# kskjs1203/SevenNet_finetuning

Hardware: AMD Instinct MI355X
Metric: atoms/sec energy+force, SevenNet-0 lmax=2, 97,336-atom box @1 GPU (higher is better)
Workload: dtype f32 (MLP / linear products on bf16 MFMA pieces: bf16x6 fwd, bf16x3 bwd); 1 GPU; SevenNet-0 energy+force+virial, 97,336-atom periodic Si box (23^3 cells), 1 GPU; total_atoms=97336, scaling=weak, atoms_per_rank=97336, edges_per_rank=2725408, parallelism=single

## Files before the change

sevennet_finetuning_amd/csrc/api.cpp:

```cpp
#include <hip/hip_runtime.h>

#include <algorithm>
#include <cmath>
#include <cstdio>
#include <cstdlib>
#include <cstring>
#include <fstream>
#include <map>
#include <memory>
#include <sstream>
#include <string>
#include <vector>

#include "../../include/e3gnn.h"
#include "bias_row.h"
#include "cg_tables.h"
#include "d3.h"
#include "dbuf.h"
#include "fcn_act.h"
#include "generic.h"
#include "train_ops.h"
#include "common.h"
#include "fused.h"
#include "gtp.h"
#include "minijson.h"
#include "node.h"
#include "neighbor.h"
#include "tgemm.h"
#include "tp.h"

using namespace e3gnn;

namespace {

thread_local std::string g_err;

int fail(int code, const std::string& msg) {
  g_err = msg;
  return code;
}

bool trace_errors() {
  static int on = [] {
    const char* v = std::getenv("E3GNN_TRACE_ERRORS");
    return v && v[0] == '1';
  }();
  return on;
}
void trace_point(const char* where) {
  if (!trace_errors()) return;
  hipError_t e = hipPeekAtLastError();
  if (e != hipSuccess) std::fprintf(stderr, "[e3gnn] sticky HIP error %d (%s) at %s\n", (int)e,
                                    hipGetErrorString(e), where);
}

#define HIPCHK(expr)                                                                          \
  do {                                                                                        \
    hipError_t _e = (expr);                                                                   \
    if (_e != hipSuccess)                                                                     \
      return fail(E3GNN_ERR_HIP, std::string(#expr) + ": " + hipGetErrorString(_e));         \
  } while (0)

struct Irr {
  int mul, l;
};
using Irreps = std::vector<Irr>;

Irreps parse_irreps(const std::string& s) {
  Irreps out;
  std::stringstream ss(s);
  std::string term;
  while (std::getline(ss, term, '+')) {
    const auto x = term.find('x');
    out.push_back({std::stoi(term.substr(0, x)), std::stoi(term.substr(x + 1))});
  }
  return out;
}
int irreps_dim(const Irreps& ir) {
  int d = 0;
  for (auto& i : ir) d += i.mul * (2 * i.l + 1);
  return d;
}
// ... 18 lines not shown
  std::memcpy(&x, &u, 4);
  return x;
}

struct LinBlock {
  int l, K, N, in_off, out_off, w_off, wt_off;
};
struct Linear {
  std::vector<LinBlock> blocks;
  DBuf W, WT;
  std::vector<float> W_h, WT_h;
  int din = 0, dout = 0;
};

struct PairBlock {
  int l, N, out_off, K1, off1, K2, off2, w_off;
  int64_t wb_off;
};
struct LinPair {
  std::vector<PairBlock> blocks;
  DBuf W;
  DBuf Wb;
  bool ok = false;
};

}

struct e3gnn_model {
  int device = 0;
  int nsp = 0, nlayer = 0;
  int family = 0;
  int kcode(int t) const { return 3 * family + (t == 0 ? 0 : (t == nlayer - 1 ? 2 : 1)); }
  std::vector<GateDims> gdims;
  int max_dx = 0, max_dg = 0;
  float cutoff = 5.f, r_on = 4.5f;
  int raw_sh = 0;
  std::vector<Irreps> irreps;
  std::vector<Irreps> gin, mid;
  std::vector<int> W;
  std::vector<float> denom;
  DBuf coeffs, embed, readout_v, scale, shift;
  std::vector<std::unique_ptr<Linear>> sc, si1, si2;
  std::vector<DBuf> b_si1, b_si2;
  bool fcn = false;
  FcnDims fcnd{};
  DBuf fcn_w;
  std::vector<std::unique_ptr<LinPair>> nl_si1, nl_si1t, nl_si2t, nl_fwd, nl_bwd;
  struct Mlp {
    DBuf w0, w1, w2, w0t, w1t, w2t;
    DBuf w1p, w2p, w2q, w2r;
    DBuf w2b;
    DBuf w2d;
    DBuf w2v;
    DBuf w1b, w1tb, w0tb;
  };
  std::vector<Mlp> mlp;
  GenModel* gen = nullptr;
  ~e3gnn_model() {
    if (gen) gen_free(gen);
  }
};

namespace {

struct Stat {
  double ms = 0, flops = 0, bytes = 0;
  int64_t launches = 0;
};
struct Pending {
  int cls;
  hipEvent_t a, b;
  double flops, bytes;
};
const char* kClassNames[] = {"graph_build", "edge_embed",  "node_linear", "radial_mlp_fwd",
                             "tp_fwd",      "gate_fwd",    "readout",     "gate_bwd",
                             "tp_bwd",      "radial_mlp_bwd", "gather_src", "edge_force",
                             "atom_force",  "embed",
                             "conv_fwd.first", "conv_fwd.mid", "conv_fwd.last",
                             "conv_bwd_x.first", "conv_bwd_x.mid", "conv_bwd_x.last"};
enum Cls {
  C_GRAPH,
  C_EMBED_EDGE,
  C_LINEAR,
  C_MLP_FWD,
  C_TP_FWD,
  C_GATE_FWD,
  C_READOUT,
  C_GATE_BWD,
  C_TP_BWD,
  C_MLP_BWD,
  C_GATHER,
  C_EDGE_FORCE,
  C_ATOM_FORCE,
  C_EMBED_NODE,
  C_CONV_FWD,
  C_CONV_BWD_X = C_CONV_FWD + 3,
  C_NCLS = C_CONV_BWD_X + 3
};
static_assert(sizeof(kClassNames) / sizeof(kClassNames[0]) == C_NCLS, "class names");

double tp_flops_per_edge(int code) { return fused_kind_tp_flops(code); }

}

struct e3gnn_ctx {
  e3gnn_model* m;
// ... 306 lines not shown
bool check_paths(int code, const Irreps& x, int lmax_out) {
  struct Ins {
    int l1, l2, l3, mul, xoff;
  };
  const auto P = kind_paths(code);
  int DX = 0, W = 0, DM = 0;
  if (P.empty() || !fused_kind_dims(code, &DX, &W, &DM)) return false;
  std::vector<Ins> ins;
  int xoff = 0;
  for (auto& i : x) {
    for (int l2 = 0; l2 <= 2; ++l2)
      for (int l3 = std::abs(i.l - l2); l3 <= i.l + l2; ++l3)
        if (l3 <= lmax_out) ins.push_back({i.l, l2, l3, i.mul, xoff});
    xoff += i.mul * (2 * i.l + 1);
  }
  if (ins.size() != P.size()) return false;
  std::vector<int> moff(ins.size());
  int off = 0;
  for (int l3 = 0; l3 <= 2; ++l3)
    for (size_t k = 0; k < ins.size(); ++k)
      if (ins[k].l3 == l3) {
        moff[k] = off;
        off += ins[k].mul * (2 * l3 + 1);
      }
  if (off != DM) return false;
  int woff = 0;
  for (size_t k = 0; k < ins.size(); ++k) {
    const PathDef& p = P[k];
    if (p.l1 != ins[k].l1 || p.l2 != ins[k].l2 || p.l3 != ins[k].l3 || p.mul != ins[k].mul ||
        p.xoff != ins[k].xoff || p.woff != woff || p.moff != moff[k])
      return false;
    woff += ins[k].mul;
  }
  return woff == W && xoff == DX;
}

}

namespace {
template <int A, int B, int C>
void dense_cg(float* out) {
  using T = CG<A, B, C>;
  std::memset(out, 0, sizeof(float) * (2 * A + 1) * (2 * B + 1) * (2 * C + 1));
  for (int q = 0; q < T::n; ++q)
    out[(T::e[q].i * (2 * B + 1) + T::e[q].j) * (2 * C + 1) + T::e[q].k] = T::e[q].c;
}
MlpW mlp_ptrs(const e3gnn_model* m, int t) {
  const auto& mm = m->mlp[t];
  return MlpW{mm.w0.f(),  mm.w1.f(),  mm.w2.f(),  mm.w2t.f(),
              mm.w1p.f(), mm.w2p.f(), mm.w2q.f(), mm.w2r.f(),
              static_cast<const uint16_t*>(mm.w2b.p),
              static_cast<const uint16_t*>(mm.w2d.p),
              static_cast<const uint16_t*>(mm.w2v.p),
              static_cast<const uint16_t*>(mm.w1b.p),
              static_cast<const uint16_t*>(mm.w1tb.p),
              static_cast<const uint16_t*>(mm.w0tb.p)};
}

}

namespace {
GenGraph gen_graph(e3gnn_ctx* c) {
  return GenGraph{c->n, c->nl, c->E, c->type.i(), c->nbr.i(), c->vec.f(), c->row_ptr.i(),
                  c->src_ptr.i(), c->src_perm.i(), c->err.i()};
}

int fused_family(const minijson::Value& man) {
  if (const char* g = std::getenv("E3GNN_GENERIC"); g && g[0] == '1') return -1;
  if (man.has("is_parity") && man["is_parity"].boolean()) return -1;
  const int lmax = man.has("lmax_edge") ? (int)man["lmax_edge"].num()
                                        : (man.has("lmax") ? (int)man["lmax"].num() : 2);
  if (lmax != 2) return -1;
  if (man.has("self_connection_type") && man["self_connection_type"].str() != "linear") return -1;
  if (!man.has("cutoff_function") || man["cutoff_function"]["name"].str() != "XPLOR") return -1;
  if (man.has("readout") && man["readout"].has("type") && man["readout"]["type"].str() != "linear") {
    const auto& ro = man["readout"];
    if (ro["type"].str() != "fcn" || !ro.has("hidden") || !ro.has("act") || !ro.has("act_norm")) return -1;
    const auto& h = ro["hidden"].arr();
    if (h.size() < 1 || h.size() > (size_t)FCN_MAX_HIDDEN) return -1;
    for (auto& w : h)
      if (w.num() < 1 || w.num() > FCN_MAX_WIDTH || w.num() != std::floor(w.num())) return -1;
    bool known = false;
    for (int k = 0; k < FCN_ACT_KINDS; ++k) known = known || ro["act"].str() == fcn_act_names()[k];
    if (!known) return -1;
  }
  const int L = (int)man["num_convolution_layer"].num();
  if (L < 2) return -1;
  if (man.has("weight_nn_hidden_neurons")) {
    const auto& h = man["weight_nn_hidden_neurons"].arr();
    if (h.size() != 2 || (int)h[0].num() != 64 || (int)h[1].num() != 64) return -1;
  }
  if (man.has("radial_basis") && man["radial_basis"].has("num") && (int)man["radial_basis"]["num"].num() != 8)
    return -1;
  const auto& ir = man["irreps_manual"].arr();
  if ((int)ir.size() != L + 1) return -1;
  Irreps first, mid, last;
  try {
    first = merged(parse_irreps(ir[0].str()));
    mid = merged(parse_irreps(ir[1].str()));
    last = merged(parse_irreps(ir[L].str()));
  } catch (...) {
    return -1;
  }
  if (first.size() != 1 || first[0].l != 0 || last.size() != 1 || last[0].l != 0) return -1;
  for (int t = 1; t < L; ++t)
    if (ir[t].str() != ir[1].str()) return -1;
// ... 267 lines not shown
              for (int q = 0; q < 4; ++q)
                for (int t = 0; t < 4; ++t)
                  o[(size_t)n * 64 + g * 16 + q * 4 + t] = a[(size_t)(16 * q + 4 * g + t) * N + n];
          return o;
        };
        std::vector<float> q2((size_t)W * 64);
        for (int cb = 0; cb < W / 16; ++cb)
          for (int bh = 0; bh < 4; ++bh)
            for (int g = 0; g < 4; ++g)
              for (int c = 0; c < 16; ++c)
                for (int sx = 0; sx < 4; ++sx)
                  q2[((size_t)(cb * 4 + bh) * 64 + g * 16 + c) * 4 + sx] =
                      a2[(size_t)(16 * bh + c) * W + 16 * cb + 4 * sx + g];
        std::vector<float> r2((size_t)W * 64);
        for (int cb = 0; cb < W / 16; ++cb)
          for (int bh = 0; bh < 4; ++bh)
            for (int g = 0; g < 4; ++g)
              for (int c = 0; c < 16; ++c)
                for (int r = 0; r < 4; ++r)
                  r2[((size_t)(cb * 4 + bh) * 64 + g * 16 + c) * 4 + r] =
                      a2[(size_t)(16 * bh + c) * W + 16 * cb + 4 * g + r];
        auto bsplit = [](const std::vector<float>& a, int N) {
          std::vector<float> o((size_t)N * 64 * 3 / 2);
          uint16_t* oh = reinterpret_cast<uint16_t*>(o.data());
          for (int cb = 0; cb < N / 16; ++cb)
            for (int m2 = 0; m2 < 2; ++m2)
              for (int g = 0; g < 4; ++g)
                for (int c = 0; c < 16; ++c)
                  for (int t = 0; t < 8; ++t) {
                    float v = a[(size_t)(16 * (2 * m2 + t / 4) + 4 * g + t % 4) * N + 16 * cb + c];
                    for (int pc = 0; pc < 3; ++pc) {
                      const uint16_t hb = bf16_rne(v);
                      oh[((((size_t)cb * 3 + pc) * 2 + m2) * 64 + g * 16 + c) * 8 + t] = hb;
                      v -= bf16_to_f32(hb);
                    }
                  }
          return o;
        };
        const std::vector<float> b2 = bsplit(a2, W);
        {
          const auto a0 = scaled(w0, 8, 64, s0, false);
          std::vector<float> a1t((size_t)64 * 64), a0t((size_t)64 * 16, 0.f);
          for (int i = 0; i < 64; ++i)
            for (int j = 0; j < 64; ++j) a1t[(size_t)j * 64 + i] = a1[(size_t)i * 64 + j];
          for (int n = 0; n < 8; ++n)
            for (int k = 0; k < 64; ++k) a0t[(size_t)k * 16 + n] = a0[(size_t)n * 64 + k];
          if (upload(mm.w1b, bsplit(a1, 64)) != hipSuccess || upload(mm.w1tb, bsplit(a1t, 64)) != hipSuccess ||
              upload(mm.w0tb, bsplit(a0t, 16)) != hipSuccess)
            throw std::runtime_error("upload mlp (w1b)");
        }
        const std::vector<int> cols = bwd_w_block_cols(m->kcode(t));
        if ((int)cols.size() * 16 != W || cols.size() % 2)
          throw std::runtime_error("dE/dw block order does not cover the weights");
        std::vector<float> d2((size_t)W * 64 * 3 / 2);
        uint16_t* d2h = reinterpret_cast<uint16_t*>(d2.data());
        for (size_t P = 0; P < cols.size() / 2; ++P)
          for (int bh = 0; bh < 4; ++bh)
            for (int g = 0; g < 4; ++g)
              for (int c = 0; c < 16; ++c)
                for (int t8 = 0; t8 < 8; ++t8) {
                  const int col = t8 < 4 ? cols[2 * P] + 4 * g + t8 : cols[2 * P + 1] + 4 * g + t8 - 4;
                  float v = a2[(size_t)(16 * bh + c) * W + col];
                  for (int pc = 0; pc < 3; ++pc) {
                    const uint16_t hb = bf16_rne(v);
                    d2h[(((P * 3 + pc) * 4 + bh) * 64 + g * 16 + c) * 8 + t8] = hb;
                    v -= bf16_to_f32(hb);
                  }
                }
        if (upload(mm.w2d, d2) != hipSuccess) throw std::runtime_error("upload mlp (w2d)");
        {
          std::vector<float> v2(b2.size());
          const size_t blk = (size_t)64 * 16 * 3 / 2;
          for (size_t k = 0; k < cols.size(); ++k)
            std::memcpy(v2.data() + k * blk, b2.data() + (size_t)(cols[k] / 16) * blk, blk * 4);
          if (upload(mm.w2v, v2) != hipSuccess) throw std::runtime_error("upload mlp (w2v)");
        }
        if (W % 16 || upload(mm.w1p, kperm(a1, 64)) != hipSuccess ||
            upload(mm.w2p, kperm(a2, W)) != hipSuccess || upload(mm.w2q, q2) != hipSuccess ||
            upload(mm.w2r, r2) != hipSuccess ||
            upload(mm.w2b, b2) != hipSuccess)
          throw std::runtime_error("upload mlp (packed)");
      }
      trace_point("load:mlp");
    }
  } catch (const std::exception& ex) {
    fail(E3GNN_ERR_IO, std::string("model load: ") + ex.what());
    return nullptr;
  }
  trace_point("load:exit");
  (void)hipGetLastError();
  return m.release();
}

void e3gnn_free(e3gnn_model* m) { delete m; }

int e3gnn_model_info(const e3gnn_model* m, int* num_species, float* cutoff, int* num_layers,
                     int* comm_size) {
  if (!m) return fail(E3GNN_ERR_ARG, "null model");
  if (num_species) *num_species = m->nsp;
  if (cutoff) *cutoff = m->cutoff;
  if (num_layers) *num_layers = m->nlayer;
  if (comm_size) {
    if (m->gen) {
      int d = 0;
      for (int t = 1; t <= m->nlayer; ++t) d = std::max(d, gen_feature_dim(m->gen, t));
      *comm_size = d;
    } else {
      *comm_size = irreps_dim(m->irreps[1]);
    }
  }
  return E3GNN_OK;
}

int64_t e3gnn_gemm_workspace_floats(int n, const e3gnn_gemm_desc* d) {
  if (n < 0 || (n > 0 && !d)) return -1;
  int64_t w = 0;
  for (int i = 0; i < n; ++i) {
    const int sp = tg_splits(d[i].m, d[i].n, (int64_t)d[i].k + d[i].k2);
    if (sp > 1) w += (int64_t)sp * d[i].m * d[i].n;
  }
  return w;
}

static int gemm_prob(const e3gnn_gemm_desc& q, int i, TgProb& p) {
  if (q.m < 0 || q.n < 0 || q.k < 0 || q.k2 < 0 || (q.m > 0 && q.n > 0 && (!q.c || (q.k > 0 && (!q.a || !q.b)) ||
                                                                      (q.k2 > 0 && (!q.a2 || !q.b2)))))
    return fail(E3GNN_ERR_ARG, "e3gnn_gemm_grouped: bad problem " + std::to_string(i));
  if (q.beta != 0 && q.beta != 1) return fail(E3GNN_ERR_ARG, "e3gnn_gemm_grouped: beta must be 0 or 1");
// ... 1877 lines not shown
```

sevennet_finetuning_amd/csrc/fused.h:

```cpp
#pragma once
#include <hip/hip_runtime.h>
#include <cstdint>

namespace e3gnn {

struct MlpW {
  const float* w0;
  const float* w1;
  const float* w2;
  const float* w2t;
  const float* w1p;
  const float* w2p;
  const float* w2q;
  const float* w2r;
  const uint16_t* w2b;
  const uint16_t* w2d;
  const uint16_t* w2v;
  const uint16_t* w1b;
  const uint16_t* w1tb;
  const uint16_t* w0tb;
};

struct FusedArgs {
  const int* row_ptr;
  const int* center;
  const int* nbr;
  const float* emb;
  const float* Y;
  const float* h;
  float* agg;
  const float* gagg;
  const int* src_ptr;
  const int* src_perm;
  float* dh;
  float* dxc;
  float* dgu;
  float* demb;
  MlpW W;
  int n_centers;
  int n_edges;
  int n_nodes;
  float denom;
  int c_begin, c_end, node_begin, node_end;
};

hipError_t launch_conv_fwd(int kind, const FusedArgs& a, hipStream_t s);
hipError_t launch_conv_bwd_ls(int kind, const FusedArgs& a, hipStream_t s);
hipError_t launch_conv_bwd_nbr_last(int kind, const FusedArgs& a, hipStream_t s);

}
```

sevennet_finetuning_amd/csrc/fused.hip:

```cpp
#include "cg_tables.h"
#include "common.h"
#include "fused.h"
#include "tp.h"

#include <type_traits>


namespace e3gnn {
namespace {

typedef float f32x4 __attribute__((ext_vector_type(4)));

template <int N, int I = 0, class F>
constexpr void sfor_host(F&& f) {
  if constexpr (I < N) {
    f(std::integral_constant<int, I>{});
    sfor_host<N, I + 1>(f);
  }
}
template <int N, int I = 0, class F>
__device__ __forceinline__ void sfor(F&& f) {
  if constexpr (I < N) {
    f(std::integral_constant<int, I>{});
    sfor<N, I + 1>(f);
  }
}

__device__ __forceinline__ constexpr int yoff(int l) { return l == 0 ? 0 : (l == 1 ? 1 : 4); }
__device__ __forceinline__ constexpr int KH(int s) { return 16 * (s >> 2) + (s & 3); }

__device__ __forceinline__ void phase() { __builtin_amdgcn_sched_barrier(0); }

#ifndef E3GNN_STAMPS_FWD
#define E3GNN_STAMPS_FWD 0
#endif
#ifdef E3GNN_STAMPS
__device__ unsigned long long* g_stamp_buf = nullptr;
#define STAMP_N 8
#define STAMP_DECL                               \
  unsigned long long st_acc[STAMP_N] = {0, 0, 0, 0, 0, 0, 0, 0}; \
  unsigned long long st_t = __builtin_amdgcn_s_memtime(), st_t0 = st_t;
#define STAMP(k)                                          \
  do {                                                    \
    const unsigned long long st_now = __builtin_amdgcn_s_memtime(); \
    st_acc[k] += st_now - st_t;                           \
    st_t = st_now;                                        \
  } while (0)
#define STAMP_FLUSH(wave)                                                   \
  do {                                                                      \
    if (g_stamp_buf && lane == 0) {                                         \
      st_acc[7] = __builtin_amdgcn_s_memtime() - st_t0;                     \
      for (int k_ = 0; k_ < STAMP_N; ++k_) g_stamp_buf[(int64_t)(wave) * STAMP_N + k_] = st_acc[k_]; \
    }                                                                       \
  } while (0)
#else
#define STAMP_DECL
// ... 676 lines not shown
    mlp_chain<CX3>(R, b, lane, m);
  }

  f32x4 dh1[4];
  {
    f32x4 da2[4];
#pragma unroll
    for (int bb = 0; bb < 4; ++bb)
#pragma unroll
      for (int r = 0; r < 4; ++r) da2[bb][r] = dh2[bb][r] * act_grad(m.a2[bb][r]);
    Op3 dq;
    split_h2(da2, dq);
#pragma unroll
    for (int bi = 0; bi < 4; ++bi) {
      phase();
      Op3 wq;
      load_w2b(wq, R.w1tb, lane, 16 * bi);
      dh1[bi] = CX3 ? w2_block3<false>(dq, wq) : w2_block<false>(dq, wq);
    }
  }
  f32x4 de;
  {
    f32x4 da1[4];
#pragma unroll
    for (int q = 0; q < 4; ++q)
#pragma unroll
      for (int t = 0; t < 4; ++t) da1[q][t] = dh1[q][t] * act_grad(m.a1[q][t]);
    Op3 dq, wq;
    split_h2(da1, dq);
    load_w2b(wq, R.w0tb, lane, 0);
    de = CX3 ? w2_block3<false>(dq, wq) : w2_block<false>(dq, wq);
  }
  if (g < 2 && er >= 0) {
    if (dold) {
#pragma unroll
      for (int r = 0; r < 4; ++r) demb[(int64_t)er * 8 + 4 * g + r] = dold[r] + de[r];
    } else {
#pragma unroll
      for (int r = 0; r < 4; ++r) demb[(int64_t)er * 8 + 4 * g + r] += de[r];
    }
  }
}
__device__ __forceinline__ void mlp_bwd_chain(const WRes& R, const float* __restrict__ emb, int e0,
                                              int end, int lane, const f32x4 (&dh2)[4],
                                              float* __restrict__ demb, const float* dold = nullptr,
                                              const float* bk = nullptr, const f32x4* a2k = nullptr) {
  const int e = e0 + (lane & 15);
  mlp_bwd_chain_ids(R, emb, e < end ? e : -1, lane, dh2, demb, dold, bk, a2k);
}

#ifndef E3GNN_DH2_X3
#define E3GNN_DH2_X3 1
#endif
constexpr int LS_BLK = 6144;
constexpr int LS_PAIR_W = 2 * LS_BLK;
constexpr int LS_PAIR_D = 12288;

__device__ __forceinline__ void dh2_pair_g2(f32x4 (&dh2)[2][4], const float (&dp)[2][4], const float (&dr)[2][4],
                                            bool two, __amdgpu_buffer_rsrc_t w2d, int pair, int lane) {
  bf16x8 d[2][2];
#pragma unroll
  for (int u = 0; u < 2; ++u) {
    float v[8];
#pragma unroll
    for (int t = 0; t < 8; ++t) v[t] = t < 4 ? dp[u][t] : dr[u][t - 4];
    split2x8(v, d[u]);
  }
  bf16x8 a[4][2];
#pragma unroll
  for (int bh = 0; bh < 4; ++bh)
#pragma unroll
    for (int pc = 0; pc < 2; ++pc)
      a[bh][pc] = __builtin_bit_cast(
          bf16x8, __builtin_amdgcn_raw_buffer_load_b128(w2d, lane * 16, pair * LS_PAIR_D + (pc * 4 + bh) * 1024, 0));
#pragma unroll
  for (int bh = 0; bh < 4; ++bh) {
#pragma unroll
    for (int u = 0; u < 2; ++u) {
      if (u == 1 && !two) break;
      dh2[u][bh] = mfma16(a[bh][1], d[u][0], dh2[u][bh]);
      dh2[u][bh] = mfma16(a[bh][0], d[u][1], dh2[u][bh]);
      dh2[u][bh] = mfma16(a[bh][0], d[u][0], dh2[u][bh]);
    }
  }
}

constexpr bool NBR_DH2_BF16 = E3GNN_DH2_X3 != 0;
template <class L>
__global__ __launch_bounds__(256) __attribute__((amdgpu_waves_per_eu(2, 2))) void k_conv_bwd_nbr(
    const int* __restrict__ src_ptr, const int* __restrict__ src_perm, const int* __restrict__ center,
    const float* __restrict__ emb, const float* __restrict__ Y, const float* __restrict__ h,
    const float* __restrict__ gagg, MlpW W, float* __restrict__ dh, float* __restrict__ dgu, int n_centers,
    int r_begin, int r_end, float* __restrict__ demb) {
  __shared__ __attribute__((aligned(16))) float lds[4][L::DX];
  const int wid = threadIdx.x >> 6;
  const int jn = __builtin_amdgcn_readfirstlane(r_begin + blockIdx.x * 4 + wid);
  if (jn >= r_end) return;
  float* dacc = lds[wid];
  const int lane = threadIdx.x & 63, g = lane >> 4, col = lane & 15;
  const int qb = src_ptr[jn], qe = src_ptr[jn + 1];
  const WRes R = make_wres(W, L::W);
  const __amdgpu_buffer_rsrc_t Rx = rsrc_bytes(h + (int64_t)jn * L::DX, L::DX * 4);
  const __amdgpu_buffer_rsrc_t Rg = rsrc_bytes(gagg, (int64_t)n_centers * L::DM * 4);
  for (int t = lane; t < L::DX; t += 64) dacc[t] = 0.f;
  const RowSel rsel = row_scatter_sel(col);
  const int own = row_scatter_own(col);

  for (int q0 = qb; q0 < qe; q0 += 32) {
// ... 119 lines not shown
                }
              }
              pin<4 * D1>(dx);
              wcur[0] = wnxt[0];
              wcur[1] = wnxt[1];
              ++nb;
            }
          });
          phase();
          {
            constexpr int NV = 4 * D1;
            static_assert(NV % 8 == 4, "batches of 16, 8, then 4");
            float* da = dacc + XOFF + (16 * jj + 4 * g) * D1;
            if constexpr (NV >= 16) da[own] += row_scatter16<16>(dx, rsel);
            if constexpr (NV % 16 >= 8) da[NV / 16 * 16 + (own & 7)] += row_scatter16<8>(dx + NV / 16 * 16, rsel);
            da[NV / 8 * 8 + (own & 3)] += row_scatter16<4>(dx + NV / 8 * 8, rsel);
          }
        }
      }
    });

#pragma unroll
    for (int u = 0; u < 2; ++u) {
      if (u == 1 && !two) break;
      phase();
      float d[8];
#pragma unroll
      for (int q = 0; q < 8; ++q) d[q] = sum_rows4(dYa[u][q + 1]);
      if (g == 0 && er[u] >= 0) {
        const float s3 = 1.7320508075688772f, s5 = 2.23606797749979f, c15 = s3 * s5;
        const float is3 = 0.57735026918962576f;
        const float ux = y[u][1] * is3, uy = y[u][2] * is3, uz = y[u][3] * is3;
        const float gx = s3 * d[0] + c15 * (uz * d[3] + uy * d[4]) - s5 * ux * d[5] - c15 * ux * d[7];
        const float gy = s3 * d[1] + c15 * (ux * d[4] + uz * d[6]) + 2.f * s5 * uy * d[5];
        const float gz = s3 * d[2] + c15 * (ux * d[3] + uy * d[6]) - s5 * uz * d[5] + c15 * uz * d[7];
        float* o = dgu + (int64_t)er[u] * 3;
        o[0] = gu_old[u][0] + gx;
        o[1] = gu_old[u][1] + gy;
        o[2] = gu_old[u][2] + gz;
      }
      phase();
      mlp_bwd_chain_ids(R, emb, er[u], lane, dh2[u], demb, de_old[u]);
    }
  }
  phase();
  __builtin_amdgcn_s_waitcnt(0);
  float* dhj = dh + (int64_t)jn * L::DX;
  for (int t = lane; t < L::DX; t += 64) dhj[t] = dacc[t];
}


constexpr int LS_WPC = E3GNN_BWD_W_X3 ? 2 : 3;
constexpr int LS_DPC = E3GNN_DH2_X3 ? 2 : 3;
constexpr int LS_IBLK = LS_WPC * 2048;
constexpr int LS_IW = 2 * LS_IBLK;
constexpr int LS_IMG = LS_IW + LS_DPC * 4096;

template <int NPC = 3>
__device__ __forceinline__ void lds_op3(Op3& o, const char* blk, int lane) {
#pragma unroll
  for (int pc = 0; pc < NPC; ++pc)
#pragma unroll
    for (int m = 0; m < 2; ++m)
      o.v[pc][m] = *reinterpret_cast<const bf16x8*>(blk + ((pc * 2 + m) * 64 + lane) * 16);
}

__device__ __forceinline__ void dh2_pair(f32x4 (&dh2)[4], const float (&da)[4], const float (&db)[4],
                                         const char* pimg, int lane) {
  if constexpr (E3GNN_DH2_X3) {
    bf16x8 d[2];
    {
      float v[8];
#pragma unroll
      for (int t = 0; t < 8; ++t) v[t] = t < 4 ? da[t] : db[t - 4];
      split2x8(v, d);
    }
    bf16x8 a[4][2];
#pragma unroll
    for (int bh = 0; bh < 4; ++bh)
#pragma unroll
      for (int pc = 0; pc < 2; ++pc)
        a[bh][pc] = *reinterpret_cast<const bf16x8*>(pimg + ((pc * 4 + bh) * 64 + lane) * 16);
    phase();
#pragma unroll
    for (int bh = 0; bh < 4; ++bh) {
      dh2[bh] = mfma16(a[bh][1], d[0], dh2[bh]);
      dh2[bh] = mfma16(a[bh][0], d[1], dh2[bh]);
      dh2[bh] = mfma16(a[bh][0], d[0], dh2[bh]);
    }
    return;
  }
  bf16x8 d[3];
  {
    float v[8];
#pragma unroll
    for (int t = 0; t < 8; ++t) v[t] = t < 4 ? da[t] : db[t - 4];
    split3x8(v, d);
  }
  constexpr int I[6] = {2, 1, 0, 1, 0, 0}, J[6] = {0, 1, 2, 0, 1, 0};
#pragma unroll
  for (int bh = 0; bh < 4; ++bh) {
    bf16x8 a[3];
#pragma unroll
    for (int pc = 0; pc < 3; ++pc)
      a[pc] = *reinterpret_cast<const bf16x8*>(pimg + ((pc * 4 + bh) * 64 + lane) * 16);
#pragma unroll
    for (int q = 0; q < 6; ++q) dh2[bh] = mfma16(a[I[q]], d[J[q]], dh2[bh]);
  }
}

__device__ __forceinline__ int ls_tiles(const int* __restrict__ row_ptr, int cb, int c_end) {
  int T = 0;
#pragma unroll
  for (int w = 0; w < 4; ++w) {
    const int cc = cb + w;
    if (cc < c_end) T = max(T, (row_ptr[cc + 1] - row_ptr[cc] + 15) >> 4);
  }
  return __builtin_amdgcn_readfirstlane(T);
}

template <class L>
struct BwdLsWaves {
  static constexpr int v = L::KIND == 0 ? 3 : 2;
};
constexpr int LS_WPG = 4;
template <class L>
struct LsTwoImages {
  static constexpr bool lean = LS_WPC == 2 && LS_DPC == 2;
  static constexpr int OFF0 = L::KIND == 1 ? L::P[0].mul : 0;
  static constexpr int DMS = L::DM - OFF0;
  static constexpr int bytes = LS_WPG * DMS * 4 + 2 * LS_IMG;
  static constexpr bool v = lean && BwdLsWaves<L>::v * bytes <= 163840;
};
template <int P>
__device__ __forceinline__ void ls_prio() { __builtin_amdgcn_s_setprio(P); }
template <class L>
__global__ __launch_bounds__(64 * LS_WPG) __attribute__((amdgpu_waves_per_eu(BwdLsWaves<L>::v, BwdLsWaves<L>::v))) void k_conv_bwd_ls(
    const int* __restrict__ row_ptr, const int* __restrict__ nbr, const float* __restrict__ emb,
    const float* __restrict__ Y, const float* __restrict__ h, const float* __restrict__ gagg, MlpW W,
    float* __restrict__ dxc, float* __restrict__ dgu, float* __restrict__ demb, int c_begin,
    int c_end, int n_nodes) {
  constexpr int NBLK = L::W / 16, NPAIR = NBLK / 2;
  static_assert(NBLK % 2 == 0, "weight blocks come in pairs");
  constexpr int WPG = LS_WPG, NT = 64 * WPG;
  constexpr int NWP = LS_IW / 16, NW = NWP / NT, NST = LS_IMG / 16 / NT, PB = LS_IBLK / 16;
  static_assert(LS_IMG / 16 % NT == 0 && NWP % NT == 0 && PB % 64 == 0, "staging pieces per thread");
  constexpr bool TWO = LsTwoImages<L>::v;
  constexpr bool KEEP = BwdLsWaves<L>::v == 2;
  constexpr int OFF0 = TWO ? LsTwoImages<L>::OFF0 : 0, DMS = L::DM - OFF0;
  static_assert(!TWO || (L::P[0].l1 == 0 && L::P[0].l2 == 0 && L::P[0].l3 == 0 && L::P[0].moff == 0 &&
                         OFF0 % 4 == 0), "path 0 is the 0e x 0e -> 0e slice at the row start");
  __shared__ __attribute__((aligned(16))) float smem[WPG * DMS + (TWO ? 2 : 1) * LS_IMG / 4];
  const int tid = threadIdx.x, wid = __builtin_amdgcn_readfirstlane(tid >> 6), lane = tid & 63, g = lane >> 4, col = lane & 15;
  const int cb = c_begin + blockIdx.x * WPG;
  const int c = cb + wid;
  const bool valid = c < c_end;
  const int beg = valid ? row_ptr[c] : 0, end = valid ? row_ptr[c + 1] : 0;
  const int T = ls_tiles(row_ptr, cb, c_end);
  float* dacc = smem + wid * DMS - OFF0;
  char* img = reinterpret_cast<char*>(smem + WPG * DMS);
  if (valid && end > beg) {
    const float4* s4 = reinterpret_cast<const float4*>(gagg + (int64_t)c * L::DM + OFF0);
    float4* d4 = reinterpret_cast<float4*>(dacc + OFF0);
    for (int k = lane; k < DMS / 4; k += 64) d4[k] = s4[k];
  }
  int rb = 0;
  const __amdgpu_buffer_rsrc_t Rg0 =
      rsrc_bytes(gagg + (valid ? (int64_t)c * L::DM : 0), valid ? (int64_t)OFF0 * 4 : 0);
  const WRes R = make_wres(W, L::W);
  const __amdgpu_buffer_rsrc_t Rx = rsrc_bytes(h, (int64_t)n_nodes * L::DX * 4);
  f32x4 st[NST];
  auto issue = [&](int P) {
    auto wsrc = [&](int idx) { return (idx / PB) * LS_BLK + (idx % PB) * 16; };
#pragma unroll
    for (int i = 0; i < NW; ++i) st[i] = ldw4(R.w2v, wsrc(tid + NT * i), P * LS_PAIR_W);
#pragma unroll
    for (int i = NW; i < NST; ++i) st[i] = ldw4(R.w2d, (tid + NT * i - NWP) * 16, P * LS_PAIR_D);
  };
  auto commit = [&]() {
    __syncthreads();
#pragma unroll
    for (int i = 0; i < NST; ++i) *reinterpret_cast<f32x4*>(img + (tid + NT * i) * 16) = st[i];
    __syncthreads();
  };
  constexpr bool STAMPED = std::is_same<L, LayerMid>::value && !E3GNN_STAMPS_FWD;
  STAMP_DECL
  issue(0);
  for (int t = 0; t < T; ++t) {
    if constexpr (STAMPED) STAMP(0);
    const int q0 = beg + 16 * t;
    const bool act = q0 < end;
    const int er = (act && q0 + col < end) ? q0 + col : -1;
    const int vx = (er >= 0 ? nbr[er] : 0) * L::DX * 4;
    float xpf[20];
    float g0pf[4];
    auto load_group = [&](auto Iq, int jq) {
      constexpr int D1q = 2 * Iq + 1;
      constexpr int XOq = iblock_xoff<L, Iq>();
      ldv<4 * D1q>(Rx, vx + 4 * g * D1q * 4, (XOq + 16 * jq * D1q) * 4, xpf);
      if constexpr (OFF0 > 0 && Iq == 0) ldv<4>(Rg0, 4 * g * 4, 16 * jq * 4, g0pf);
    };
    float y[9];
    float gu_old[3] = {0.f, 0.f, 0.f}, de_old[4] = {0.f, 0.f, 0.f, 0.f};
    f32x4 a2k[4];
    float bk[2];
    Op3 hq;
    load_group(std::integral_constant<int, first_I<L>()>{}, 0);
    const int nrow = (act && dxc) ? min(16, end - q0) : 0;
    const __amdgpu_buffer_rsrc_t Rd =
        rsrc_bytes(dxc ? dxc + (int64_t)(act ? q0 : 0) * L::DX : gagg, (int64_t)nrow * L::DX * 4);
    const int vd = col * L::DX * 4;
    if (act) {
#pragma unroll
      for (int q = 0; q < 9; ++q) y[q] = er >= 0 ? Y[(int64_t)er * 9 + q] : 0.f;
      float b[2];
#pragma unroll
      for (int s = 0; s < 2; ++s) b[s] = er >= 0 ? emb[(int64_t)er * 8 + 4 * s + g] : 0.f;
      if constexpr (KEEP) {
        if (g == 0 && er >= 0) {
#pragma unroll
          for (int k = 0; k < 3; ++k) gu_old[k] = dgu[(int64_t)er * 3 + k];
        }
        if (g < 2 && er >= 0) {
#pragma unroll
          for (int k = 0; k < 4; ++k) de_old[k] = demb[(int64_t)er * 8 + 4 * g + k];
        }
      }
      MlpT m;
      mlp_chain<CX3>(R, b, lane, m);
      if constexpr (KEEP) {
// ... 16 lines not shown
    for (int q = 0; q < 9; ++q) dYa[q] = 0.f;
    float dwp[4];
    f32x4 wv0 = zero4(), wv1 = zero4();
    sfor<3>([&](auto I) {
      constexpr int MUL = iblock_mul<L, I>();
      if constexpr (MUL > 0) {
        constexpr int D1 = 2 * I + 1;
        constexpr int XOFF = iblock_xoff<L, I>();
        constexpr int NPI = paths_of<L>(I), U = (NPI & 1) ? 2 : 1, NB0 = blocks_before<L>(I);
        static_assert((MUL / 16) % U == 0, "channel groups come in pairs");
        for (int j2 = 0; j2 < MUL / 16; j2 += U) {
          sfor<U>([&](auto hh) {
            const int jj = j2 + hh;
            float x[4 * D1], dx[4 * D1], g0[4];
#pragma unroll
            for (int i = 0; i < 4 * D1; ++i) {
              x[i] = xpf[i];
              dx[i] = 0.f;
            }
            if constexpr (OFF0 > 0 && I == 0) {
#pragma unroll
              for (int i = 0; i < 4; ++i) g0[i] = g0pf[i];
            }
            if (jj + 1 < MUL / 16) {
              load_group(I, jj + 1);
            } else {
              constexpr int IN = next_I<L>(I);
              if constexpr (IN >= 0) load_group(std::integral_constant<int, IN>{}, 0);
            }
            sfor<L::NP>([&](auto pi) {
              constexpr PathDef p = L::P[pi];
              if constexpr (p.l1 == I) {
                constexpr int D3 = 2 * p.l3 + 1;
                constexpr int ODD = (NB0 + hh * NPI + path_rank<L>(pi)) & 1;
                const int nb = NB0 + jj * NPI + path_rank<L>(pi);
                const char* pimg = img + (TWO ? rb * LS_IMG : 0);
                if constexpr (!ODD) {
                  if constexpr (STAMPED) STAMP(5);
                  const int nextP = (nb >> 1) + 1 < NPAIR ? (nb >> 1) + 1 : 0;
                  if constexpr (TWO) {
#pragma unroll
                    for (int i = 0; i < NST; ++i)
                      *reinterpret_cast<f32x4*>(img + rb * LS_IMG + (tid + NT * i) * 16) = st[i];
                    __syncthreads();
                    issue(nextP);
                  } else {
                    commit();
                    issue(nextP);
                  }
                  if constexpr (STAMPED) STAMP(2);
                  if (act) {
                    ls_prio<1>();
                    Op3 wq, wq1;
                    lds_op3<LS_WPC>(wq, pimg, lane);
                    lds_op3<LS_WPC>(wq1, pimg + LS_IBLK, lane);
                    phase();
                    wv0 = w2_block_bwd<false>(hq, wq);
                    wv1 = w2_block_bwd<false>(hq, wq1);
                    ls_prio<0>();
                  }
                  if constexpr (STAMPED) STAMP(3);
                }
                if (act) {
                  const f32x4 wv = ODD ? wv1 : wv0;
                  float gm[4 * D3];
                  if constexpr (OFF0 > 0 && pi == 0) {
#pragma unroll
                    for (int k = 0; k < 4; ++k) gm[k] = g0[k];
                  } else {
                    const float* gl = dacc + p.moff + 16 * jj * D3 + 4 * g * D3;
#pragma unroll
                    for (int k = 0; k < 4 * D3; ++k) gm[k] = gl[k];
                  }
                  float dwr[4];
                  tp_bwd_xw4<p.l1, p.l2, p.l3>(x, y + yoff(p.l2), wv, gm, dx, dYa + yoff(p.l2), dwr);
                  if constexpr (L::KIND != 0) pin<4 * D1>(dx);
                  pin<8>(dYa + 1);
                  if constexpr (ODD) {
                    if constexpr (STAMPED) STAMP(5);
                    ls_prio<1>();
                    dh2_pair(dh2, dwp, dwr, pimg + LS_IW, lane);
                    ls_prio<0>();
                    if constexpr (STAMPED) STAMP(4);
                  } else {
#pragma unroll
                    for (int r = 0; r < 4; ++r) dwp[r] = dwr[r];
                  }
                }
                if constexpr (TWO && ODD) rb ^= 1;
              }
            });
            if constexpr (L::KIND != 0)
              stv<4 * D1>(Rd, vd + 4 * g * D1 * 4, (XOFF + 16 * jj * D1) * 4, dx);
          });
        }
      }
    });
    if (act) {
      {
        float d4a[4] = {dYa[1], dYa[2], dYa[3], dYa[4]}, d4b[4] = {dYa[5], dYa[6], dYa[7], dYa[8]};
        sum_rows4_n<4>(d4a);
        sum_rows4_n<4>(d4b);
#pragma unroll
        for (int q = 0; q < 4; ++q) {
          dYa[1 + q] = d4a[q];
          dYa[5 + q] = d4b[q];
        }
      }
      if (g == 0 && er >= 0) {
        const float s3 = 1.7320508075688772f, s5 = 2.23606797749979f, c15 = s3 * s5;
        const float is3 = 0.57735026918962576f;
        const float ux = y[1] * is3, uy = y[2] * is3, uz = y[3] * is3;
        const float* d = dYa + 1;
        const float gx = s3 * d[0] + c15 * (uz * d[3] + uy * d[4]) - s5 * ux * d[5] - c15 * ux * d[7];
        const float gy = s3 * d[1] + c15 * (ux * d[4] + uz * d[6]) + 2.f * s5 * uy * d[5];
        const float gz = s3 * d[2] + c15 * (ux * d[3] + uy * d[6]) - s5 * uz * d[5] + c15 * uz * d[7];
        float* o = dgu + (int64_t)er * 3;
        if constexpr (KEEP) {
          o[0] = gu_old[0] + gx;
          o[1] = gu_old[1] + gy;
          o[2] = gu_old[2] + gz;
        } else {
          o[0] += gx;
          o[1] += gy;
          o[2] += gz;
        }
      }
      if constexpr (STAMPED) STAMP(5);
      mlp_bwd_chain(R, emb, q0, end, lane, dh2, demb, KEEP ? de_old : nullptr, KEEP ? bk : nullptr,
                    KEEP ? a2k : nullptr);
    }
    if constexpr (STAMPED) STAMP(6);
  }
  if constexpr (STAMPED) STAMP_FLUSH(blockIdx.x * WPG + wid);
// ... 143 lines not shown
```

Baseline: 2.510 million atoms/s.

## Share one swizzled W2 image for both backward uses via transposed LDS reads

Instead of staging two separate W2 copies per weight pair (a transposed one for dE/dw and a row-major one for dh2), a single swizzled bf16x3 image is packed at load time. The backward kernel reads it row-wise for dh2 and with ds_read_tr16_b64 transposed reads for the w2 block product. This cuts global traffic and LDS footprint per pair, and it also enables double-buffered images for more layers now that the lean restriction is gone. The cost is extra LDS read instructions and more complex addressing. The old w2d/w2v path is kept only for kcode%3==2.

```diff
diff --git a/sevennet_finetuning_amd/csrc/api.cpp b/sevennet_finetuning_amd/csrc/api.cpp
--- a/sevennet_finetuning_amd/csrc/api.cpp
+++ b/sevennet_finetuning_amd/csrc/api.cpp
@@ -28,6 +28,7 @@
 #include "neighbor.h"
 #include "tgemm.h"
 #include "tp.h"
+#include "w2_image.h"
 
 using namespace e3gnn;
 
@@ -152,6 +153,7 @@
     DBuf w2b;
     DBuf w2d;
     DBuf w2v;
+    DBuf w2s;
     DBuf w1b, w1tb, w0tb;
   };
   std::vector<Mlp> mlp;
@@ -564,6 +566,7 @@
               static_cast<const uint16_t*>(mm.w2b.p),
               static_cast<const uint16_t*>(mm.w2d.p),
               static_cast<const uint16_t*>(mm.w2v.p),
+              static_cast<const uint16_t*>(mm.w2s.p),
               static_cast<const uint16_t*>(mm.w1b.p),
               static_cast<const uint16_t*>(mm.w1tb.p),
               static_cast<const uint16_t*>(mm.w0tb.p)};
@@ -937,28 +940,33 @@
         const std::vector<int> cols = bwd_w_block_cols(m->kcode(t));
         if ((int)cols.size() * 16 != W || cols.size() % 2)
           throw std::runtime_error("dE/dw block order does not cover the weights");
-        std::vector<float> d2((size_t)W * 64 * 3 / 2);
-        uint16_t* d2h = reinterpret_cast<uint16_t*>(d2.data());
-        for (size_t P = 0; P < cols.size() / 2; ++P)
-          for (int bh = 0; bh < 4; ++bh)
-            for (int g = 0; g < 4; ++g)
-              for (int c = 0; c < 16; ++c)
-                for (int t8 = 0; t8 < 8; ++t8) {
-                  const int col = t8 < 4 ? cols[2 * P] + 4 * g + t8 : cols[2 * P + 1] + 4 * g + t8 - 4;
-                  float v = a2[(size_t)(16 * bh + c) * W + col];
-                  for (int pc = 0; pc < 3; ++pc) {
-                    const uint16_t hb = bf16_rne(v);
-                    d2h[(((P * 3 + pc) * 4 + bh) * 64 + g * 16 + c) * 8 + t8] = hb;
-                    v -= bf16_to_f32(hb);
+        if (m->kcode(t) % 3 == 2) {
+          std::vector<float> d2((size_t)W * 64 * 3 / 2);
+          uint16_t* d2h = reinterpret_cast<uint16_t*>(d2.data());
+          for (size_t P = 0; P < cols.size() / 2; ++P)
+            for (int bh = 0; bh < 4; ++bh)
+              for (int g = 0; g < 4; ++g)
+                for (int c = 0; c < 16; ++c)
+                  for (int t8 = 0; t8 < 8; ++t8) {
+                    const int col = t8 < 4 ? cols[2 * P] + 4 * g + t8 : cols[2 * P + 1] + 4 * g + t8 - 4;
+                    float v = a2[(size_t)(16 * bh + c) * W + col];
+                    for (int pc = 0; pc < 3; ++pc) {
+                      const uint16_t hb = bf16_rne(v);
+                      d2h[(((P * 3 + pc) * 4 + bh) * 64 + g * 16 + c) * 8 + t8] = hb;
+                      v -= bf16_to_f32(hb);
+                    }
                   }
-                }
-        if (upload(mm.w2d, d2) != hipSuccess) throw std::runtime_error("upload mlp (w2d)");
-        {
+          if (upload(mm.w2d, d2) != hipSuccess) throw std::runtime_error("upload mlp (w2d)");
           std::vector<float> v2(b2.size());
           const size_t blk = (size_t)64 * 16 * 3 / 2;
           for (size_t k = 0; k < cols.size(); ++k)
             std::memcpy(v2.data() + k * blk, b2.data() + (size_t)(cols[k] / 16) * blk, blk * 4);
           if (upload(mm.w2v, v2) != hipSuccess) throw std::runtime_error("upload mlp (w2v)");
+        } else {
+          const size_t npairs = cols.size() / 2;
+          std::vector<float> s2(npairs * w2img::PAIR_BYTES / 4);
+          w2img::pack(a2.data(), W, cols.data(), (int)npairs, reinterpret_cast<uint16_t*>(s2.data()));
+          if (upload(mm.w2s, s2) != hipSuccess) throw std::runtime_error("upload mlp (w2s)");
         }
         if (W % 16 || upload(mm.w1p, kperm(a1, 64)) != hipSuccess ||
             upload(mm.w2p, kperm(a2, W)) != hipSuccess || upload(mm.w2q, q2) != hipSuccess ||
diff --git a/sevennet_finetuning_amd/csrc/fused.h b/sevennet_finetuning_amd/csrc/fused.h
--- a/sevennet_finetuning_amd/csrc/fused.h
+++ b/sevennet_finetuning_amd/csrc/fused.h
@@ -16,6 +16,7 @@
   const uint16_t* w2b;
   const uint16_t* w2d;
   const uint16_t* w2v;
+  const uint16_t* w2s;
   const uint16_t* w1b;
   const uint16_t* w1tb;
   const uint16_t* w0tb;
diff --git a/sevennet_finetuning_amd/csrc/fused.hip b/sevennet_finetuning_amd/csrc/fused.hip
--- a/sevennet_finetuning_amd/csrc/fused.hip
+++ b/sevennet_finetuning_amd/csrc/fused.hip
@@ -2,6 +2,7 @@
 #include "common.h"
 #include "fused.h"
 #include "tp.h"
+#include "w2_image.h"
 
 #include <type_traits>
 
@@ -784,8 +785,6 @@
 #ifndef E3GNN_DH2_X3
 #define E3GNN_DH2_X3 1
 #endif
-constexpr int LS_BLK = 6144;
-constexpr int LS_PAIR_W = 2 * LS_BLK;
 constexpr int LS_PAIR_D = 12288;
 
 __device__ __forceinline__ void dh2_pair_g2(f32x4 (&dh2)[2][4], const float (&dp)[2][4], const float (&dr)[2][4],
@@ -1011,17 +1010,14 @@
 
 constexpr int LS_WPC = E3GNN_BWD_W_X3 ? 2 : 3;
 constexpr int LS_DPC = E3GNN_DH2_X3 ? 2 : 3;
-constexpr int LS_IBLK = LS_WPC * 2048;
-constexpr int LS_IW = 2 * LS_IBLK;
-constexpr int LS_IMG = LS_IW + LS_DPC * 4096;
+constexpr int LS_IMG = (LS_WPC > LS_DPC ? LS_WPC : LS_DPC) * w2img::PIECE_BYTES;
 
 template <int NPC = 3>
-__device__ __forceinline__ void lds_op3(Op3& o, const char* blk, int lane) {
+__device__ __forceinline__ void lds_op3(Op3& o, const char* pimg, int b, int lane) {
 #pragma unroll
   for (int pc = 0; pc < NPC; ++pc)
 #pragma unroll
-    for (int m = 0; m < 2; ++m)
-      o.v[pc][m] = *reinterpret_cast<const bf16x8*>(blk + ((pc * 2 + m) * 64 + lane) * 16);
+    for (int m = 0; m < 2; ++m) o.v[pc][m] = w2img::tr_read(pimg, lane, b, pc, m);
 }
 
 __device__ __forceinline__ void dh2_pair(f32x4 (&dh2)[4], const float (&da)[4], const float (&db)[4],
@@ -1039,7 +1035,7 @@
     for (int bh = 0; bh < 4; ++bh)
 #pragma unroll
       for (int pc = 0; pc < 2; ++pc)
-        a[bh][pc] = *reinterpret_cast<const bf16x8*>(pimg + ((pc * 4 + bh) * 64 + lane) * 16);
+        a[bh][pc] = w2img::row_read(pimg, lane, pc, bh);
     phase();
 #pragma unroll
     for (int bh = 0; bh < 4; ++bh) {
@@ -1062,7 +1058,7 @@
     bf16x8 a[3];
 #pragma unroll
     for (int pc = 0; pc < 3; ++pc)
-      a[pc] = *reinterpret_cast<const bf16x8*>(pimg + ((pc * 4 + bh) * 64 + lane) * 16);
+      a[pc] = w2img::row_read(pimg, lane, pc, bh);
 #pragma unroll
     for (int q = 0; q < 6; ++q) dh2[bh] = mfma16(a[I[q]], d[J[q]], dh2[bh]);
   }
@@ -1085,11 +1081,10 @@
 constexpr int LS_WPG = 4;
 template <class L>
 struct LsTwoImages {
-  static constexpr bool lean = LS_WPC == 2 && LS_DPC == 2;
   static constexpr int OFF0 = L::KIND == 1 ? L::P[0].mul : 0;
   static constexpr int DMS = L::DM - OFF0;
   static constexpr int bytes = LS_WPG * DMS * 4 + 2 * LS_IMG;
-  static constexpr bool v = lean && BwdLsWaves<L>::v * bytes <= 163840;
+  static constexpr bool v = BwdLsWaves<L>::v * bytes <= 163840;
 };
 template <int P>
 __device__ __forceinline__ void ls_prio() { __builtin_amdgcn_s_setprio(P); }
@@ -1102,8 +1097,8 @@
   constexpr int NBLK = L::W / 16, NPAIR = NBLK / 2;
   static_assert(NBLK % 2 == 0, "weight blocks come in pairs");
   constexpr int WPG = LS_WPG, NT = 64 * WPG;
-  constexpr int NWP = LS_IW / 16, NW = NWP / NT, NST = LS_IMG / 16 / NT, PB = LS_IBLK / 16;
-  static_assert(LS_IMG / 16 % NT == 0 && NWP % NT == 0 && PB % 64 == 0, "staging pieces per thread");
+  constexpr int NST = LS_IMG / 16 / NT;
+  static_assert(LS_IMG / 16 % NT == 0, "staging pieces per thread");
   constexpr bool TWO = LsTwoImages<L>::v;
   constexpr bool KEEP = BwdLsWaves<L>::v == 2;
   constexpr int OFF0 = TWO ? LsTwoImages<L>::OFF0 : 0, DMS = L::DM - OFF0;
@@ -1127,14 +1122,12 @@
   const __amdgpu_buffer_rsrc_t Rg0 =
       rsrc_bytes(gagg + (valid ? (int64_t)c * L::DM : 0), valid ? (int64_t)OFF0 * 4 : 0);
   const WRes R = make_wres(W, L::W);
+  const __amdgpu_buffer_rsrc_t Rs = rsrc_bytes(W.w2s, NPAIR * w2img::PAIR_BYTES);
   const __amdgpu_buffer_rsrc_t Rx = rsrc_bytes(h, (int64_t)n_nodes * L::DX * 4);
   f32x4 st[NST];
   auto issue = [&](int P) {
-    auto wsrc = [&](int idx) { return (idx / PB) * LS_BLK + (idx % PB) * 16; };
-#pragma unroll
-    for (int i = 0; i < NW; ++i) st[i] = ldw4(R.w2v, wsrc(tid + NT * i), P * LS_PAIR_W);
-#pragma unroll
-    for (int i = NW; i < NST; ++i) st[i] = ldw4(R.w2d, (tid + NT * i - NWP) * 16, P * LS_PAIR_D);
+#pragma unroll
+    for (int i = 0; i < NST; ++i) st[i] = ldw4(Rs, (tid + NT * i) * 16, P * w2img::PAIR_BYTES);
   };
   auto commit = [&]() {
     __syncthreads();
@@ -1257,8 +1250,8 @@
                   if (act) {
                     ls_prio<1>();
                     Op3 wq, wq1;
-                    lds_op3<LS_WPC>(wq, pimg, lane);
-                    lds_op3<LS_WPC>(wq1, pimg + LS_IBLK, lane);
+                    lds_op3<LS_WPC>(wq, pimg, 0, lane);
+                    lds_op3<LS_WPC>(wq1, pimg, 1, lane);
                     phase();
                     wv0 = w2_block_bwd<false>(hq, wq);
                     wv1 = w2_block_bwd<false>(hq, wq1);
@@ -1284,7 +1277,7 @@
                   if constexpr (ODD) {
                     if constexpr (STAMPED) STAMP(5);
                     ls_prio<1>();
-                    dh2_pair(dh2, dwp, dwr, pimg + LS_IW, lane);
+                    dh2_pair(dh2, dwp, dwr, pimg, lane);
                     ls_prio<0>();
                     if constexpr (STAMPED) STAMP(4);
                   } else {
diff --git a/sevennet_finetuning_amd/csrc/w2_image.h b/sevennet_finetuning_amd/csrc/w2_image.h
--- /dev/null
+++ b/sevennet_finetuning_amd/csrc/w2_image.h
@@ -0,0 +1,71 @@
+#pragma once
+#include <cstdint>
+#include <cstring>
+
+namespace e3gnn {
+namespace w2img {
+
+constexpr int ROWS = 64;
+constexpr int ROW_BYTES = 64;
+constexpr int PIECE_BYTES = ROWS * ROW_BYTES;
+constexpr int PIECES = 3;
+constexpr int PAIR_BYTES = PIECES * PIECE_BYTES;
+
+constexpr int swz(int h) { return (((h >> 3) & 1) << 2) | ((h >> 2) & 1); }
+constexpr int off(int pc, int h, int u) { return pc * PIECE_BYTES + h * ROW_BYTES + 8 * (u ^ swz(h)); }
+
+inline uint16_t bf16_rne(float x) {
+  uint32_t u;
+  std::memcpy(&u, &x, 4);
+  u += 0x7fffu + ((u >> 16) & 1u);
+  return (uint16_t)(u >> 16);
+}
+inline float bf16_to_f32(uint16_t h) {
+  const uint32_t u = (uint32_t)h << 16;
+  float x;
+  std::memcpy(&x, &u, 4);
+  return x;
+}
+
+inline void pack(const float* a2, int W, const int* cols, int npairs, uint16_t* out) {
+  for (int P = 0; P < npairs; ++P)
+    for (int h = 0; h < ROWS; ++h)
+      for (int b = 0; b < 2; ++b)
+        for (int ch = 0; ch < 16; ++ch) {
+          float v = a2[(size_t)h * W + cols[2 * P + b] + ch];
+          for (int pc = 0; pc < PIECES; ++pc) {
+            const uint16_t hb = bf16_rne(v);
+            out[((size_t)P * PAIR_BYTES + off(pc, h, 2 * (ch >> 2) + b)) / 2 + (ch & 3)] = hb;
+            v -= bf16_to_f32(hb);
+          }
+        }
+}
+
+#if defined(__HIPCC__)
+typedef __bf16 bf16x8 __attribute__((ext_vector_type(8)));
+typedef short s16x4 __attribute__((ext_vector_type(4)));
+typedef short s16x8 __attribute__((ext_vector_type(8)));
+
+__device__ __forceinline__ bf16x8 row_read(const char* img, int lane, int pc, int bh) {
+  const int g = lane >> 4, c = lane & 15;
+  const int a0 = off(0, c, 2 * g), a1 = a0 ^ 8;
+  const int k = pc * PIECE_BYTES + 16 * bh * ROW_BYTES;
+  typedef const volatile __attribute__((address_space(3))) s16x4* lds_vp;
+  const s16x4 lo = *(lds_vp)(img + a0 + k);
+  const s16x4 hi = *(lds_vp)(img + a1 + k);
+  return __builtin_bit_cast(bf16x8, __builtin_shufflevector(lo, hi, 0, 1, 2, 3, 4, 5, 6, 7));
+}
+
+__device__ __forceinline__ bf16x8 tr_read(const char* img, int lane, int b, int pc, int m) {
+  const int g = lane >> 4, q = (lane >> 2) & 3, p = lane & 3;
+  const int a = off(0, 4 * g + q, 2 * p) ^ (8 * b);
+  const int k = pc * PIECE_BYTES + 32 * m * ROW_BYTES;
+  typedef __attribute__((address_space(3))) s16x4* lds_p;
+  const s16x4 lo = __builtin_amdgcn_ds_read_tr16_b64_v4i16((lds_p)(img + a + k));
+  const s16x4 hi = __builtin_amdgcn_ds_read_tr16_b64_v4i16((lds_p)(img + a + k + 16 * ROW_BYTES));
+  return __builtin_bit_cast(bf16x8, __builtin_shufflevector(lo, hi, 0, 1, 2, 3, 4, 5, 6, 7));
+}
+#endif
+
+}
+}
```

Measured after the change: 2.558 million atoms/s, median of 6. 1.9% higher.
